# geoHeil/splink

Hardware: AMD Instinct MI355X
Metric: candidate pairs scored/sec (gammas+E+M per iter) (higher is better)
Workload: dtype fp64; 1 GPU; cfg2: synthetic person-record dedupe, 1M x sqrt(N) records, blocking surname|dob, 5 comparison columns (JW-3 x2, exact-2 x2, Levenshtein-3); records=1000000, candidate_pairs=45981122, comparison_columns=5, candidate_ordinals_total=46222173, comparison_windows=2, parallelism=pair-ordinal shards x1, RCCL all-reduce of pattern histogram

## Files before the change

### include/splink_hip.h

```cpp
#ifndef SPLINK_HIP_H
#define SPLINK_HIP_H

#include <stdint.h>

#ifdef __cplusplus
extern "C" {
#endif

#define SPK_OK 0
#define SPK_E_INVALID (-1)
#define SPK_E_HIP (-2)
#define SPK_E_OOM (-3)
#define SPK_E_STATE (-4)
#define SPK_E_LIMIT (-5)

#define SPK_LINK_DEDUPE 0
#define SPK_LINK_ONLY 1
#define SPK_LINK_AND_DEDUPE 2

typedef struct spk_ctx spk_ctx;

const char *spk_last_error(void);
int spk_version(void);
int spk_device_count(int *out);
// ... 100 lines not shown
                       const int32_t *rule_program, int shard, int n_shards, int n_cols,
                       const spk_column_program *cols, int n_when, const int32_t *when_first_instr,
                       const int32_t *when_n_instr, const int32_t *when_level, int n_instr,
                       const spk_instr *instr, int n_operands, const spk_operand *operands, int n_lits,
                       const int64_t *lit_offsets, const uint8_t *lit_utf8, int64_t *out_n_pairs,
                       int64_t *out_n_candidates_total);
int spk_block_residual_info(spk_ctx *ctx, int64_t *out_enumerated, double *out_filter_ms);
int spk_gammas_copy(spk_ctx *ctx, int64_t start, int64_t count, int8_t *out);
int spk_gammas_load(spk_ctx *ctx, int n_cols, const int32_t *n_levels, int64_t n, const int8_t *gammas);
int spk_n_patterns(spk_ctx *ctx, int64_t *out);
int spk_gammas_deferred(spk_ctx *ctx, int64_t *out);
int spk_gammas_exact_counts(spk_ctx *ctx, int64_t *out, int n);
int spk_gammas_exact_ms(spk_ctx *ctx, double *out, int n);
int spk_gammas_exact_list(spk_ctx *ctx, int k, int32_t *out, int64_t n);
int spk_gammas_implied_pairs(spk_ctx *ctx, int64_t *out, int n);
int spk_gammas_set_simple(spk_ctx *ctx, int on);
int spk_gammas_simple_count(spk_ctx *ctx, int *out);
int spk_gammas_set_window(spk_ctx *ctx, int64_t pairs);
int spk_gammas_windows(spk_ctx *ctx, int64_t *out);
int spk_gammas_set_streams(spk_ctx *ctx, int streams, int64_t min_pairs);
int spk_gammas_set_graph(spk_ctx *ctx, int on);
int spk_gammas_graph_launches(spk_ctx *ctx, int64_t *out);
int spk_gammas_set_lev_kernel(spk_ctx *ctx, int mode);
int spk_gammas_view_regions(spk_ctx *ctx, int64_t *out);

int spk_jaro_winkler_sim(spk_ctx *ctx, int64_t n, const int64_t *l_offsets, const uint8_t *l_utf8,
                         const int64_t *r_offsets, const uint8_t *r_utf8, double *out);
int spk_levenshtein(spk_ctx *ctx, int64_t n, const int64_t *l_offsets, const uint8_t *l_utf8,
                    const int64_t *r_offsets, const uint8_t *r_utf8, double *out);

int spk_em_iteration(spk_ctx *ctx, double lambda, double one_minus, const double *m, const double *u,
                     double *out_stats, int n_stats);
int spk_em_iteration_start(spk_ctx *ctx, double lambda, double one_minus, const double *m, const double *u,
                           int n_stats);
int spk_em_iteration_wait(spk_ctx *ctx, double *out_stats, int n_stats);
int spk_em_histogram(spk_ctx *ctx, uint64_t *d_hist);
int spk_em_set_lane_histogram(spk_ctx *ctx, int on);
int spk_em_finalize(spk_ctx *ctx, const uint64_t *d_hist, double lambda, double one_minus, const double *m,
                    const double *u, double *out_stats, int n_stats);
int spk_em_histogram_async(spk_ctx *ctx, uint64_t *d_hist);
int spk_em_finalize_start(spk_ctx *ctx, const uint64_t *d_hist, double lambda, double one_minus, const double *m,
                          const double *u, int n_stats);
int spk_score(spk_ctx *ctx, double lambda, double one_minus, const double *m, const double *u, int64_t start,
              int64_t count, double *out_mp);

#define SPK_SEL_MP 0
// ... 58 lines not shown
```

### splink_amd/_native.py

```python
from __future__ import annotations

import ctypes
import os

import numpy as np

_HERE = os.path.dirname(os.path.abspath(__file__))
LIB_PATH = os.environ.get("SPLINK_AMD_LIB", os.path.join(_HERE, "libsplink_hip.so"))

SPK_OK = 0
SPK_E_INVALID = -1
SPK_E_HIP = -2
SPK_E_OOM = -3
SPK_E_STATE = -4
SPK_E_LIMIT = -5

LINK_TYPES = {"dedupe_only": 0, "link_only": 1, "link_and_dedupe": 2}

OPERAND_DTYPE = np.dtype([("kind", "<i4"), ("side", "<i4"), ("col", "<i4"), ("lit", "<i4"), ("num", "<f8"),
                          ("has_num_default", "<i4"), ("substr_start", "<i4"), ("substr_len", "<i4"),
                          ("pad", "<i4")], align=True)
INSTR_DTYPE = np.dtype([("op", "<i4"), ("a", "<i4"), ("b", "<i4"), ("cmp", "<i4"), ("i0", "<i4"), ("pad", "<i4"),
                        ("t", "<f8")], align=True)
PROGRAM_DTYPE = np.dtype([("n_levels", "<i4"), ("else_level", "<i4"), ("n_when", "<i4"), ("first_when", "<i4")],
# ... 10 lines not shown
SELECT_CHUNK = 2048
COMPONENTS_CHUNK = 1024
assert OPERAND_DTYPE.itemsize == 40 and INSTR_DTYPE.itemsize == 32 and PROGRAM_DTYPE.itemsize == 16

OP = {"ISNULL": 1, "NOTNULL": 2, "STR_CMP": 3, "NUM_CMP": 4, "JW": 5, "LEV": 6, "LEVRATIO": 7, "ABSDIFF": 8,
      "PERCDIFF": 9, "CONST": 10, "LEN": 11, "AND": 20, "OR": 21, "NOT": 22}
CMP = {"=": 0, "==": 0, "!=": 1, "<>": 1, "<": 2, "<=": 3, ">": 4, ">=": 5}

EXPORTS = [
    "spk_last_error", "spk_version", "spk_device_count", "spk_ctx_create", "spk_ctx_destroy", "spk_ctx_set_stream",
    "spk_ctx_sync", "spk_ctx_set_link_type", "spk_ctx_kernel_ms", "spk_ctx_enable_timing", "spk_table_create",
    "spk_table_add_utf8", "spk_table_add_float64", "spk_table_set_rank", "spk_table_set_key", "spk_block",
    "spk_pairs_count", "spk_pairs_copy", "spk_pairs_load", "spk_gammas", "spk_gammas_copy", "spk_gammas_load",
    "spk_n_patterns", "spk_gammas_deferred", "spk_em_histogram", "spk_em_finalize", "spk_em_iteration", "spk_score",
    "spk_tf_accumulate", "spk_tf_apply", "spk_jaro_winkler_sim", "spk_levenshtein", "spk_gammas_exact_counts",
    "spk_gammas_set_simple", "spk_gammas_exact_list", "spk_gammas_simple_count", "spk_em_set_lane_histogram", "spk_table_set_rank_null",
    "spk_gammas_view_regions", "spk_ctx_lds_per_block", "spk_ctx_memory", "spk_raw_utf8", "spk_raw_i64", "spk_key_build", "spk_rank_from_raw", "spk_cluster", "spk_table_add_raw_utf8",
    "spk_gammas_implied_pairs", "spk_tf_column_values", "spk_tf_accumulate_column", "spk_tf_apply_columns", "spk_tf_copy", "spk_tf_set_mode",
    "spk_tf_accumulate_exact", "spk_tf_accumulate_column_exact", "spk_tf_limbs_to_sum", "spk_tf_scales",
    "spk_tf_scales_column", "spk_raw_utf8_arrow", "spk_raw_utf8_arrow_chunks", "spk_table_digest", "spk_raw_release",
    "spk_em_iteration_start", "spk_em_iteration_wait", "spk_ctx_kernel_ms_done", "spk_em_histogram_async",
    "spk_em_finalize_start", "spk_gammas_exact_ms", "spk_gammas_set_window", "spk_gammas_windows", "spk_gammas_set_streams", "spk_gammas_set_graph",
    "spk_gammas_graph_launches",
    "spk_gammas_set_lev_kernel",
    "spk_block_residual", "spk_block_residual_info",
    "spk_select", "spk_select_copy", "spk_select_info", "spk_select_release",
    "spk_components", "spk_components_edges", "spk_components_copy", "spk_components_info", "spk_components_release",
]
TF_LIMBS = 14


class NativeUnavailable(RuntimeError):
    """libsplink_hip.so or a gfx950 HIP device is unavailable (there is no CPU fallback)."""


_lib = None


def load_library():
    global _lib
    if _lib is not None:
        return _lib
    if not os.path.exists(LIB_PATH):
        raise NativeUnavailable(f"{LIB_PATH} not found: build it with `python -c 'import __graft_entry__ as g; g.build()'`")
    lib = ctypes.CDLL(LIB_PATH)
    lib.spk_last_error.restype = ctypes.c_char_p
    lib.spk_ctx_destroy.restype = None
# ... 309 lines not shown
    def gammas_set_window(self, pairs: int):
        check(self._lib.spk_gammas_set_window(self._h, ctypes.c_int64(int(pairs))), "spk_gammas_set_window")

    def gammas_set_streams(self, streams: int, min_pairs: int = 1 << 22):
        check(self._lib.spk_gammas_set_streams(self._h, ctypes.c_int(int(streams)), ctypes.c_int64(int(min_pairs))),
              "spk_gammas_set_streams")

    def gammas_set_graph(self, on: bool):
        check(self._lib.spk_gammas_set_graph(self._h, ctypes.c_int(1 if on else 0)), "spk_gammas_set_graph")

    def gammas_graph_launches(self) -> int:
        n = ctypes.c_int64(0)
        check(self._lib.spk_gammas_graph_launches(self._h, ctypes.byref(n)), "spk_gammas_graph_launches")
        return n.value

    def gammas_windows(self) -> int:
        n = ctypes.c_int64(0)
        check(self._lib.spk_gammas_windows(self._h, ctypes.byref(n)), "spk_gammas_windows")
        return n.value

    def gammas_set_lev_kernel(self, mode: int):
        check(self._lib.spk_gammas_set_lev_kernel(self._h, ctypes.c_int(int(mode))), "spk_gammas_set_lev_kernel")

    def lds_per_block(self) -> int:
        n = ctypes.c_int(0)
        check(self._lib.spk_ctx_lds_per_block(self._h, ctypes.byref(n)), "spk_ctx_lds_per_block")
        return n.value

    MEMORY_PARTS = ("raw_columns", "record_encodings", "row_images", "pairs", "codes", "work_lists", "em_score_tf",
                    "total")

    def memory(self) -> dict:
        out = np.zeros(8, dtype=np.int64)
        check(self._lib.spk_ctx_memory(self._h, _ptr(out)), "spk_ctx_memory")
        return dict(zip(self.MEMORY_PARTS, [int(x) for x in out]))

    def gammas_view_regions(self) -> int:
        n = ctypes.c_int64(0)
        check(self._lib.spk_gammas_view_regions(self._h, ctypes.byref(n)), "spk_gammas_view_regions")
        return n.value

    def gammas_exact_ms(self, n: int):
        out = np.zeros(max(n, 1), dtype=np.float64)
        check(self._lib.spk_gammas_exact_ms(self._h, _ptr(out), ctypes.c_int(n)), "spk_gammas_exact_ms")
        return out[:n].tolist()

# ... 237 lines not shown
```

### splink_amd/csrc/spk_ctx.hip

```cpp
#include <algorithm>
#include <cstring>

#include "spk_internal.h"

namespace spk {

static thread_local std::string g_last_error;
void set_error(const std::string &msg) { g_last_error = msg; }

Table::~Table() {
    for (Column *c : cols) delete c;
    for (int w = 0; w < 2; ++w)
        for (DevBuf<int64_t> *k : key[w]) delete k;
}

int ensure_desc(spk_ctx *ctx, Table &t) {
    if (!t.desc_dirty && t.d_desc.p) return SPK_OK;
    std::vector<ColDesc> h(t.cols.size());
    for (size_t i = 0; i < t.cols.size(); ++i) {
        Column *c = t.cols[i];
        ColDesc d{};
        d.kind = c ? c->kind : COL_NONE;
        if (c && c->kind == COL_STR) {
            d.units = c->units.p;
            d.meta = c->meta.p;
            d.planes = c->planes.p;
            d.planes_hi = c->planes_hi.n ? c->planes_hi.p : nullptr;
            d.bag = c->bag.n ? c->bag.p : nullptr;
        } else if (c && c->kind == COL_NUM) {
            d.val = c->val.p;
            d.valid = c->valid.p;
        }
        h[i] = d;
    }
    SPK_TRY(t.d_desc.alloc(h.size() ? h.size() : 1));
    if (!h.empty())
        SPK_HIP(hipMemcpyAsync(t.d_desc.p, h.data(), h.size() * sizeof(ColDesc), hipMemcpyHostToDevice, ctx->stream));
    SPK_HIP(hipStreamSynchronize(ctx->stream));
    t.desc_dirty = false;
    return SPK_OK;
}


__global__ void k_utf8_decode(int64_t n, const int64_t *__restrict__ off8, const int64_t *__restrict__ src_off,
                              const int32_t *__restrict__ perm, const uint8_t *__restrict__ bytes,
                              const uint8_t *__restrict__ valid, uint16_t *__restrict__ units,
                              RecMeta *__restrict__ meta, uint64_t *__restrict__ planes,
                              uint64_t *__restrict__ planes_hi, const int64_t *__restrict__ ids) {
    int64_t row = (int64_t)blockIdx.x * blockDim.x + threadIdx.x;
    if (row >= n) return;
    const int64_t src = perm ? (int64_t)perm[row] : row;
// ... 174 lines not shown
            }
            const int sh = (b & 7) * 4;
            const uint32_t x = w[b >> 3];
            if (((x >> sh) & 15u) < 15u) w[b >> 3] = x + (1u << sh);
        }
        w[7] |= (other << 16) | ((uint32_t)len << 24);
    } else {
        w[7] = 0xFF000000u;
    }
    bag[2 * row] = make_uint4(w[0], w[1], w[2], w[3]);
    bag[2 * row + 1] = make_uint4(w[4], w[5], w[6], w[7]);
}

int build_bag_rows(spk_ctx *ctx, int64_t n, Column *c) {
    SPK_TRY(c->bag.alloc((size_t)(2 * n + 2)));
    if (n > 0) {
        k_bag_rows<<<(unsigned)((n + BAG_THREADS - 1) / BAG_THREADS), BAG_THREADS, 0, ctx->stream>>>(n, c->meta.p,
                                                                                                  c->units.p, c->bag.p);
        SPK_HIP(hipGetLastError());
    }
    return SPK_OK;
}

int launch_unit_bits(spk_ctx *ctx, int64_t n, Column *c) {
    c->unit_bits = false;
    c->bag.release();
    if (n <= 0) return SPK_OK;
    DevBuf<unsigned int> d;
    SPK_TRY(d.alloc(2));
    const unsigned int init[2] = {0u, 0xFFu};
    SPK_HIP(hipMemcpyAsync(d.p, init, sizeof(init), hipMemcpyHostToDevice, ctx->stream));
    const int64_t blocks = std::min<int64_t>((n + 255) / 256, 4 * (int64_t)ctx->n_cu);
    k_unit_bits<<<(unsigned)blocks, 256, 0, ctx->stream>>>(n, c->meta.p, c->planes.p, c->planes_hi.p, d.p);
    SPK_HIP(hipGetLastError());
    unsigned int h[2];
    SPK_HIP(hipMemcpyAsync(h, d.p, sizeof(h), hipMemcpyDeviceToHost, ctx->stream));
    SPK_HIP(hipStreamSynchronize(ctx->stream));
    c->unit_or = h[0];
    c->unit_and = h[1];
    c->unit_bits = true;
    return SPK_OK;
}

int launch_utf8_decode(spk_ctx *ctx, int64_t n, const int64_t *off8, const int64_t *src_off, const int32_t *perm,
                       const uint8_t *bytes, const uint8_t *valid, Column *c, bool long_rows, const int64_t *ids) {
    if (n <= 0) return SPK_OK;
    k_utf8_decode<<<(unsigned)((n + 255) / 256), 256, 0, ctx->stream>>>(n, off8, src_off, perm, bytes, valid, c->units.p,
                                                                        c->meta.p, c->planes.p,
                                                                        long_rows ? c->planes_hi.p : nullptr, ids);
// ... 428 lines not shown
```

### splink_amd/csrc/spk_filter.hip

```cpp
#include <algorithm>
#include <cmath>
#include <cstring>

#include "spk_gamma.h"

namespace spk {

enum LevKind : int32_t { LK_GE = 0, LK_LE = 1, LK_EXACT = 2, LK_RATIO = 3 };

struct FCommon {
    int64_t p0, p1;
    uint32_t in;
    uint32_t stride;
    int32_t k;
    int32_t null_level;
    int64_t imp_lo, imp_hi;
    uint32_t imp_add;
    int32_t und_same;
    int ws;
};

struct FEq {
    FCommon c;
    int32_t lv_same, lv_diff;
    int32_t eq4;
};

struct FJw {
    FCommon c;
    int64_t h0, h1;
    int32_t lv_one, lv_zero, lv_bound;
    float cf;
    int32_t geq;
    FEq ge[2];
};

struct FLev {
    FCommon c;
    int32_t lv_same, lv_same_empty, lv_else;
    int32_t n;
    int32_t kind[MAX_TESTS], a[MAX_TESTS], cmp[MAX_TESTS], level[MAX_TESTS];
    double t[MAX_TESTS];
};

struct FNum {
    FCommon c;
    int32_t null_level, else_level, n_tests;
    int32_t op[MAX_TESTS], cmp[MAX_TESTS], level[MAX_TESTS];
    double t[MAX_TESTS];
};

struct FiltArgs {
    const int32_t *pl, *pr;
    const uint8_t *img0, *img1;
    uint32_t plane0, plane1;
    void *codes;
    int32_t *work;
    unsigned int *region_count;
    int64_t P, region_len;
    int n_regions, region_base;
    const int16_t *thr;
    int n_thr;
    int nj, nl, ne, nn;
// ... 136 lines not shown
#pragma unroll
    for (int u = 0; u < FP; ++u) {
        const bool sat = lf[u] >= LEN_SAT || ls[u] >= LEN_SAT;
        const bool exact = same[u] || zero[u];
        const uint32_t add = same[u] ? (lf[u] > 0 ? a_one : a_zero) : (zero[u] ? a_zero : a_bound);
        const bool u0 = (same[u] && und_same) || sat || (!exact && hi[u] >= J.cf);
        und[u] = act[u] && !nul[u] && u0;
        acc[u] += und[u] ? 0u : (nul[u] ? a_null : add);
    }
}
template <int FP>
__device__ __attribute__((always_inline)) inline void f_jw(const FiltArgs &A, const FJw &J, const uint32_t (&ox)[FP],
                                                           const uint32_t (&oy)[FP], const bool (&act)[FP],
                                                           uint32_t (&acc)[FP], bool (&und)[FP]) {
    JwData<FP> d;
    ld_jw<FP>(A, J, ox, oy, d);
    ev_jw<FP>(J, d, act, acc, und);
}

template <int FP>
struct Data16 {
    uint4 a[FP], b[FP];
};
template <int FP>
__device__ __attribute__((always_inline)) inline void ev_lev(const FLev &L, const int16_t *s_thr, const Data16<FP> &d,
                                                             const bool (&act)[FP], uint32_t (&acc)[FP], bool (&und)[FP]) {
    const uint4(&a)[FP] = d.a;
    const uint4(&b)[FP] = d.b;
    bool same[FP], nul[FP], bmp[FP], u0[FP];
    int lo[FP], hi[FP], S[FP];
    bool need = false;
#pragma unroll
    for (int u = 0; u < FP; ++u) {
        same[u] = a[u].x == b[u].x && a[u].y == b[u].y;
        nul[u] = a[u].y == LENS_NULL || b[u].y == LENS_NULL;
        const int la = lens_u16(a[u].y), lb = lens_u16(b[u].y), na = lens_cp(a[u].y), nb = lens_cp(b[u].y);
        u0[u] = (same[u] && L.c.und_same) || la >= LEN_SAT || lb >= LEN_SAT || na >= LEN_SAT || nb >= LEN_SAT;
        bmp[u] = na == la && nb == lb && !same[u] && !nul[u];
        need = need || bmp[u];
        lo[u] = na > nb ? na - nb : nb - na;
        hi[u] = na > nb ? na : nb;
        S[u] = na + nb;
    }
    if (__any(need)) {
#pragma unroll
        for (int u = 0; u < FP; ++u) {
            const int na = lens_cp(a[u].y), nb = lens_cp(b[u].y);
            const int bag = hi[u] - sketch_inter_ub_bf(img_sketch(a[u]), img_sketch(b[u]), na, nb);
            lo[u] = (bmp[u] && bag > lo[u]) ? bag : lo[u];
        }
    }
    Chain ch[FP];
#pragma unroll
    for (int u = 0; u < FP; ++u) ch[u] = Chain(L.lv_else);
    bool fast = (L.n == 1 || L.n == 2) && L.kind[0] == LK_RATIO && L.a[0] >= 0 &&
                (L.n == 1 || (L.kind[1] == LK_RATIO && L.a[1] >= 0));
    if (fast) {
        bool narrow = true;
#pragma unroll
        for (int u = 0; u < FP; ++u) narrow = narrow && S[u] < THR_S;
        fast = !__any(!narrow);
    }
    if (fast) {
        const int a0 = L.a[0], lv0 = L.level[0];
#pragma unroll
// ... 305 lines not shown
    common(s, A, s.off, J.c);
    J.h0 = (int64_t)(s.off2 >> 4) * A.img_rows0 * 16;
    J.h1 = (int64_t)(s.off2 >> 4) * A.img_rows1 * 16;
    auto first_pass = [&](double v) {
        for (int i = 0; i < s.n_tests; ++i)
            if (hcmp(v, s.t[i], s.cmp[i])) return s.level[i];
        return s.else_level;
    };
    J.lv_one = first_pass(1.0);
    J.lv_zero = first_pass(0.0);
    J.lv_bound = s.else_level;
    J.cf = INFINITY;
    for (int i = 0; i < s.n_tests; ++i) {
        if (hcmp(0.0, s.t[i], s.cmp[i])) {
            J.lv_bound = s.level[i];
            break;
        }
        J.cf = std::min(J.cf, s.jw_cf[i]);
    }
}

static void make_lev(const SimpleCol &s, const GammaArgs &A, FLev &L) {
    common(s, A, s.off, L.c);
    auto same_level = [&](bool empty) {
        for (int i = 0; i < s.n_tests; ++i) {
            const int op = s.op[i];
            bool r;
            if (op == SPK_OP_STR_CMP) r = s.cmp[i] == SPK_CMP_EQ;
            else if (op == SPK_OP_LEV) r = hcmp(0.0, s.t[i], s.cmp[i]);
            else r = !empty && hcmp(0.0, s.t[i], s.cmp[i]);
            if (r) return s.level[i];
        }
        return s.else_level;
    };
    L.lv_same = same_level(false);
    L.lv_same_empty = same_level(true);
    L.n = 0;
    L.lv_else = s.else_level;
    for (int i = 0; i < s.n_tests; ++i) {
        const int op = s.op[i];
        if (op == SPK_OP_STR_CMP) {
            if (s.cmp[i] == SPK_CMP_EQ) continue;
            L.lv_else = s.level[i];
            break;
        }
        const int n = L.n++;
// ... 102 lines not shown
```

### splink_amd/csrc/spk_gamma.h

```cpp
#pragma once

#include <vector>

#include "spk_strsim.h"

namespace spk {

constexpr int F_THREADS = 256;
constexpr int X_THREADS = 256;
constexpr int U_THREADS = 128;

enum Mode { M_FILTER = 0, M_EXACT = 1, M_SLOW = 2, M_HUGE = 3 };
enum Status { ST_DONE = 0, ST_UNDECIDED = 1, ST_NEEDS_SLOW = 2 };

constexpr int MAX_TESTS = 6;
constexpr int MAX_SIMPLE = 64;
enum SimpleKind : int32_t { SK_STR = 1, SK_NUM = 2 };
enum SimpleClass : int32_t { SC_NONE = 0, SC_EQ = 1, SC_JW = 2, SC_LEV = 3, SC_NUM = 4 };
struct SimpleCol {
    int32_t k;
    int32_t kind;
    int32_t col;
    int32_t null_level, else_level, n_tests;
    int32_t op[MAX_TESTS], cmp[MAX_TESTS], level[MAX_TESTS];
    double t[MAX_TESTS];
    int64_t stride;
    int32_t cls;
    int32_t off;
    int32_t off2;
    int32_t has_ids;
    int32_t eq4;
    int32_t tflag[MAX_TESTS];
    int32_t lev_a[MAX_TESTS];
    float jw_cf[MAX_TESTS];
    int64_t imp_lo, imp_hi;
    int32_t eq_level;
    int32_t thr_off[MAX_TESTS];
    int32_t np;
};
constexpr int THR_S = 256;
constexpr int32_t TF_ZERO = 1;
constexpr int32_t TF_ONE = 2;
constexpr int32_t TF_GE = 4;
constexpr int32_t TF_EXACT = 8;
constexpr int32_t TF_EQ = 16;

constexpr int IMG_MAX = 256;
constexpr int64_t VIEW_MIN_IMAGE_BYTES = (int64_t)192 << 20;
constexpr uint32_t LENS_NULL = 0xFFFFFFFFu;
constexpr int LEN_SAT = 0xFFFE;
typedef uint32_t u32x4_t __attribute__((ext_vector_type(4)));
typedef uint32_t u32x2_t __attribute__((ext_vector_type(2)));
__device__ inline __amdgpu_buffer_rsrc_t image_rsrc(const uint8_t *base, int64_t bytes) {
    return __builtin_amdgcn_make_buffer_rsrc((void *)base, (short)0, (int)bytes, 0x00020000);
}
constexpr int64_t IMG_MAX_ROWS = ((int64_t)1 << 27) - 1;

__host__ __device__ inline int64_t img_at(int64_t rows, int64_t row, int off) {
    return ((int64_t)(off >> 4) * rows + row) * 16 + (off & 15);
}

// ... 205 lines not shown
```

### splink_amd/csrc/spk_gamma.hip

```cpp
#include <chrono>
#include <cstdio>
#include <algorithm>
#include <cstring>
#include <type_traits>
#include <cmath>

#include "spk_gamma.h"

namespace spk {

__device__ inline void apply_substr(StrView &s, int pos, int len) {
    int nc = s.ncp;
    int start = pos > 0 ? pos - 1 : (pos < 0 ? nc + pos : 0);
    long end = (long)start + len;
    if (start < 0) start = 0;
    if (end > nc) end = nc;
    s.has_meta = 0;
    s.planes = nullptr;
    if (start >= end) {
        s.n = 0;
        s.ncp = 0;
        return;
    }
    if (s.ncp == s.n) {
// ... 314 lines not shown
            }
        }
        if (r == KU) return ST_UNDECIDED;
        if (r == KT) {
            level = sc.level[i];
            return ST_DONE;
        }
    }
    level = sc.else_level;
    return ST_DONE;
}

__global__ void k_build_image(int64_t n, const ColDesc *__restrict__ cols, const SimpleCol *__restrict__ simple,
                              int n_simple, uint8_t *__restrict__ img, int64_t rows_img) {
    const int64_t row = (int64_t)blockIdx.x * blockDim.x + threadIdx.x;
    if (row >= n) return;
    for (int j = 0; j < n_simple; ++j) {
        const SimpleCol &sc = simple[j];
        const ColDesc &c = cols[sc.col];
        if (sc.cls == SC_NUM) {
            const bool ok = c.valid[row] != 0;
            *reinterpret_cast<double *>(img + img_at(rows_img, row, sc.off)) = ok ? c.val[row] : 0.0;
            *reinterpret_cast<uint2 *>(img + img_at(rows_img, row, sc.off + 8)) = make_uint2(ok ? 1u : 0u, 0u);
            continue;
        }
        const RecMeta m = c.meta[row];
        uint32_t lens = LENS_NULL;
        if (m.len16 >= 0) {
            const int l16 = m.len16 < LEN_SAT ? m.len16 : LEN_SAT;
            const int lcp = meta_cplen(m) < LEN_SAT ? meta_cplen(m) : LEN_SAT;
            lens = (uint32_t)l16 | ((uint32_t)lcp << 16);
        }
        if (sc.eq4) {
            *reinterpret_cast<uint32_t *>(img + img_at(rows_img, row, sc.off)) = m.len16 < 0 ? 0xFFFFFFFFu : m.key;
            continue;
        }
        *reinterpret_cast<uint2 *>(img + img_at(rows_img, row, sc.off)) = make_uint2(m.key, lens);
        if (sc.cls != SC_EQ) *reinterpret_cast<uint64_t *>(img + img_at(rows_img, row, sc.off + 8)) = m.sketch;
        if (sc.cls == SC_JW) *reinterpret_cast<uint64_t *>(img + img_at(rows_img, row, sc.off2)) = m.head;
    }
}

__global__ __launch_bounds__(F_THREADS) void k_gamma_filter(GammaArgs A) {
    __shared__ unsigned int s_cnt[MAX_SIMPLE];
    for (int i = threadIdx.x; i < A.n_complex; i += F_THREADS) s_cnt[i] = 0;
    __syncthreads();
// ... 1538 lines not shown
    return SPK_OK;
}

static int build_images(spk_ctx *ctx, Table &t0, Table &t1, GammaArgs &A, int64_t stride,
                        const std::vector<SimpleCol> &simple) {
    A.img0 = A.img1 = nullptr;
    A.img_stride = stride;
    if (stride <= 0 || A.n_simple == 0) return SPK_OK;
    Table *ts[2] = {&t0, &t1};
    for (int s = 0; s < 2; ++s) {
        if (s == 1 && &t1 == &t0) {
            A.img1 = A.img0;
            A.img_rows1 = A.img_rows0;
            break;
        }
        Table &t = *ts[s];
        std::vector<int64_t> key = {(int64_t)t.version, t.n, stride};
        for (const SimpleCol &sc : simple) {
            key.push_back(sc.cls);
            key.push_back(sc.col);
            key.push_back(sc.off);
            key.push_back(sc.off2);
            key.push_back(sc.eq4);
        }
        const bool fresh = ctx->img[s].p && ctx->img_key[s] == key;
        SPK_TRY(ctx->img[s].alloc((size_t)(t.n + 1) * (size_t)stride));
        ctx->img_key[s] = key;
        if (t.n > 0 && !fresh) {
            k_build_image<<<(unsigned)((t.n + 255) / 256), 256, 0, ctx->stream>>>(t.n, t.d_desc.p, A.simple, A.n_simple,
                                                                                 ctx->img[s].p, t.n + 1);
            SPK_HIP(hipGetLastError());
        }
        (s == 0 ? A.img0 : A.img1) = ctx->img[s].p;
        (s == 0 ? A.img_rows0 : A.img_rows1) = t.n + 1;
    }
    return SPK_OK;
}

static bool classify_simple(int k, const spk_column_program &prog, const int32_t *wf, const int32_t *wn,
                            const int32_t *wl, const spk_instr *instr, const spk_operand *ops, const Table &t0,
                            const Table &t1, const std::vector<int64_t> &stride, SimpleCol *out) {
    if (prog.n_when < 1 || prog.n_when - 1 > MAX_TESTS) return false;
    const int w0 = prog.first_when;
    if (wn[w0] != 3) return false;
    const spk_instr *n = instr + wf[w0];
    if (n[0].op != SPK_OP_ISNULL || n[1].op != SPK_OP_ISNULL || n[2].op != SPK_OP_OR) return false;
// ... 449 lines not shown
            const uint32_t all = t0.cols[sc.col]->unit_and & t1.cols[sc.col]->unit_and;
            while (sc.np > 5 && (((any ^ all) >> (sc.np - 1)) & 1u) == 0) --sc.np;
        }
        sc.has_ids = (t0.cols[sc.col]->has_ids && t1.cols[sc.col]->has_ids) ? 1 : 0;
        implied_equal(ctx, t0, t1, sc);
    }
    if (ctx->lev_bag) {
        bool built[2] = {false, false};
        for (const SimpleCol &sc : simple) {
            if (sc.cls != SC_LEV || sc.kind != SK_STR || !t0.cols[sc.col]->planes_hi.n || !t1.cols[sc.col]->planes_hi.n)
                continue;
            for (int s = 0; s < 2; ++s) {
                Table &t = s ? t1 : t0;
                Column *c = t.cols[sc.col];
                if (c->kind != COL_STR || c->bag.n || t.n <= 0) continue;
                SPK_TRY(build_bag_rows(ctx, t.n, c));
                t.desc_dirty = true;
                built[s] = true;
            }
        }
        if (built[0]) SPK_TRY(ensure_desc(ctx, t0));
        if (built[1]) SPK_TRY(ensure_desc(ctx, t1));
    }
    std::vector<int16_t> thr_tab;
    for (SimpleCol &sc : simple) {
        for (int i = 0; i < MAX_TESTS; ++i) sc.thr_off[i] = -1;
        if (sc.cls != SC_LEV) continue;
        for (int i = 0; i < sc.n_tests; ++i) {
            if (sc.op[i] != SPK_OP_LEVRATIO || (sc.cmp[i] != SPK_CMP_LE && sc.cmp[i] != SPK_CMP_LT)) continue;
            sc.thr_off[i] = (int32_t)thr_tab.size();
            for (int S = 0; S < THR_S; ++S) {
                int th = -1;
                const double den = (double)S / 2.0;
                for (int v = 0; v < THR_S && S > 0; ++v)
                    if (host_cmp((double)v / den, sc.t[i], sc.cmp[i])) th = v;
                    else break;
                thr_tab.push_back((int16_t)th);
            }
        }
    }
    const int64_t img_stride = layout_image(simple);
    for (size_t i = 0; i < simple.size();) {
        if (simple[i].cls == SC_NONE) {
            complex_k.push_back(simple[i].k);
            simple.erase(simple.begin() + (long)i);
        } else {
// ... 143 lines not shown
        for (const Column *c : t->cols)
            if (c && c->kind == COL_STR) G.max_units = std::max<int64_t>(G.max_units, c->max_bytes);
    for (int i = 0; i < n_lits; ++i) G.max_units = std::max<int64_t>(G.max_units, llen[i]);

    ctx->exact_carry.clear();
    ctx->deferred_carry = 0;
    ctx->last_windows = n_win;
    ctx->last_split = split;
    ctx->split_w = split ? W : 0;
    SPK_TRY(ctx->begin(K_GAMMA));
    ViewLaunch V{};
    bool have_view = false;
    ctx->last_view_regions = 0;
    if (P > 0) {
        SPK_TRY(build_images(ctx, t0, t1, A, img_stride, simple));
        const bool big = (A.img_rows0 + A.img_rows1) * img_stride > VIEW_MIN_IMAGE_BYTES;
        if ((ctx->use_views == 1 && big) || ctx->use_views == 2) SPK_TRY(build_view_images(ctx, A, img_stride, &V, &have_view));
    }
    std::vector<int64_t> gkey;
    {
        auto ptr = [](const void *q) { return (int64_t)(uintptr_t)q; };
        gkey = {P, n_win, split ? 1 : 0, W, K, ctx->code_bytes, (int64_t)ctx->pairs_epoch, (int64_t)ctx->table_epoch,
                (int64_t)std::hash<std::string>()(std::string(blob.begin(), blob.end())), ctx->lev_kernel,
                ctx->lev_bag ? 1 : 0, ctx->filter_mode, ctx->use_views, ctx->slow_force_skip ? 1 : 0,
                have_view ? 1 : 0, ptr(ctx->stream), ptr(ctx->codes.p), ptr(ctx->pl.p), ptr(ctx->pr.p), ptr(ctx->pvl.p),
                ptr(ctx->prog_blob.p), ptr(ctx->img[0].p), ptr(ctx->img[1].p), ptr(ctx->work.p), ptr(ctx->xlist.p),
                ptr(ctx->xinfo.p), ptr(ctx->xpref.p), ptr(ctx->region_count.p), ctx->xcap, ptr(ctx->alt.work.p),
                ptr(ctx->alt.xlist.p), ptr(ctx->alt.xinfo.p), ptr(ctx->alt.xpref.p), ptr(ctx->alt.region_count.p),
                ctx->alt.xcap, ptr(ctx->alt.stream), ctx->slow_seen_valid ? 1 : 0, (int64_t)ctx->timing};
        for (uint8_t f : ctx->slow_seen) gkey.push_back(f);
        for (int v = 0; v < MAX_VIEWS; ++v) gkey.push_back(ptr(ctx->vimg[v][0].p));
    }
    const bool graphable = ctx->use_graph && !ctx->timing_exact && P > 0 && fresh_blob && (split || n_win == 1);
    const bool replay = graphable && ctx->gexec && gkey == ctx->gkey;
    const bool capture = graphable && !replay && gkey == ctx->gkey_prev;
    ctx->gkey_prev = gkey;
    if (split && !replay) {
        if (!ctx->alt.gplan) ctx->alt.gplan = new GammaPlan();
        *ctx->alt.gplan = G;
    }
    bool via_graph = replay;
    if (replay) {
        ctx->gplan->slow_skipped = ctx->gskip0;
        if (split) ctx->alt.gplan->slow_skipped = ctx->gskip1;
        ctx->last_view_regions = ctx->gview_regions;
        SPK_HIP(hipGraphLaunch(ctx->gexec, ctx->stream));
        ++ctx->graph_launches;
// ... 411 lines not shown
}

extern "C" int spk_gammas_set_simple(spk_ctx *ctx, int on) {
    SPK_REQUIRE(ctx && on >= 0 && on % 10 <= 1 && on % 100 < 30 && on < 200, SPK_E_INVALID,
                "spk_gammas_set_simple: mode 0, 1 (+10 / +20) (+100)");
    ctx->use_views = on % 100 >= 20 ? 2 : (on % 100 >= 10 ? 0 : 1);
    ctx->filter_mode = on % 10;
    ctx->slow_force_skip = on >= 100;
    return SPK_OK;
}

extern "C" int spk_ctx_memory(spk_ctx *ctx, int64_t *out8) {
    SPK_REQUIRE(ctx && out8, SPK_E_INVALID, "spk_ctx_memory: null arg");
    auto b = [](const auto &buf) { return (int64_t)(buf.n * sizeof(*buf.p)); };
    int64_t m[8] = {0, 0, 0, 0, 0, 0, 0, 0};
    for (const RawCol *r : ctx->raw)
        if (r) m[0] += b(r->off) + b(r->bytes) + b(r->i64) + b(r->valid);
    for (const Table &t : ctx->table) {
        m[1] += b(t.perm) + b(t.rank) + b(t.d_desc);
        for (int w = 0; w < 2; ++w)
            for (const DevBuf<int64_t> *k : t.key[w])
                if (k) m[1] += b(*k);
        for (const Column *c : t.cols)
            if (c) m[1] += b(c->units) + b(c->meta) + b(c->planes) + b(c->planes_hi) + b(c->bag) + b(c->val) + b(c->valid);
    }
    for (int s = 0; s < 2; ++s) {
        m[2] += b(ctx->img[s]);
        for (int v = 0; v < MAX_VIEWS; ++v) m[2] += b(ctx->vimg[v][s]);
    }
    m[3] = b(ctx->pl) + b(ctx->pr) + b(ctx->pvl) + b(ctx->pvr);
    for (int v = 0; v < MAX_VIEWS; ++v) m[3] += b(ctx->views[v].rowsL) + b(ctx->views[v].rowsR);
    m[4] = b(ctx->codes);
    m[5] = b(ctx->work) + b(ctx->xlist) + b(ctx->xpref) + b(ctx->xinfo) + b(ctx->region_count) + b(ctx->prog_blob) +
           b(ctx->alt.work) + b(ctx->alt.xlist) + b(ctx->alt.xpref) + b(ctx->alt.xinfo) + b(ctx->alt.region_count);
    m[6] = b(ctx->hist) + b(ctx->mpat) + b(ctx->llpat) + b(ctx->cpat) + b(ctx->stats) + b(ctx->mu) + b(ctx->em_ticket) +
           b(ctx->em_row) + b(ctx->em_hot) + b(ctx->mp) + b(ctx->mpat_score) + b(ctx->tf_uniq) + b(ctx->tf_runs) +
           b(ctx->tf_nruns) + b(ctx->tf_mp) + b(ctx->tf_hist) +
           b(ctx->tf_sort) +
           b(ctx->sel.ord) + b(ctx->sel.l) + b(ctx->sel.r) + b(ctx->sel.code) + b(ctx->sel.mpat) +
           b(ctx->comp.label);
    for (int i = 0; i < 7; ++i) m[7] += m[i];
    for (int i = 0; i < 8; ++i) out8[i] = m[i];
    return SPK_OK;
}

extern "C" int spk_ctx_lds_per_block(spk_ctx *ctx, int *out) {
    SPK_REQUIRE(ctx && out, SPK_E_INVALID, "null arg");
// ... 34 lines not shown

extern "C" int spk_gammas_set_streams(spk_ctx *ctx, int streams, int64_t min_pairs) {
    SPK_REQUIRE(ctx && (streams == 1 || streams == 2) && min_pairs >= 0, SPK_E_INVALID,
                "spk_gammas_set_streams: 1 or 2 streams, min_pairs >= 0");
    SPK_TRY(settle_gammas(ctx, nullptr));
    ctx->gamma_streams = streams;
    ctx->split_min = min_pairs;
    return SPK_OK;
}

extern "C" int spk_gammas_windows(spk_ctx *ctx, int64_t *out) {
    SPK_REQUIRE(ctx && out, SPK_E_INVALID, "spk_gammas_windows: bad args");
    *out = ctx->last_windows;
    return SPK_OK;
}

extern "C" int spk_gammas_set_lev_kernel(spk_ctx *ctx, int mode) {
    SPK_REQUIRE(ctx && mode >= 0 && mode <= 3, SPK_E_INVALID, "spk_gammas_set_lev_kernel: mode 0 .. 3");
    ctx->lev_kernel = mode == 3 ? 2 : mode;
    ctx->lev_bag = mode != 3;
    return SPK_OK;
}

#ifdef SPK_LEVQ_STATS
extern "C" int spk_debug_levq_stats(uint64_t *out, int reset) {
    SPK_HIP(hipDeviceSynchronize());
    SPK_HIP(hipMemcpyFromSymbol(out, HIP_SYMBOL(g_levq), sizeof(uint64_t) * 16));
    if (reset) {
        static const unsigned long long zero[16] = {};
        SPK_HIP(hipMemcpyToSymbol(HIP_SYMBOL(g_levq), zero, sizeof(zero)));
    }
    return SPK_OK;
}
#endif
```

### splink_amd/csrc/spk_internal.h

```cpp
#pragma once

#include <hip/hip_runtime.h>

#include <cstdint>
#include <string>
#include <utility>
#include <vector>

#include "../../include/splink_hip.h"

namespace spk {

void set_error(const std::string &msg);

#define SPK_HIP(expr)                                                                         \
    do {                                                                                      \
        hipError_t _e = (expr);                                                               \
        if (_e != hipSuccess) {                                                               \
            ::spk::set_error(std::string(#expr) + ": " + hipGetErrorString(_e));              \
            return _e == hipErrorOutOfMemory ? SPK_E_OOM : SPK_E_HIP;                         \
        }                                                                                     \
    } while (0)

#define SPK_REQUIRE(cond, code, msg)                                                          \
// ... 28 lines not shown
__host__ __device__ inline int32_t meta_cplen(const RecMeta &m) { return (int32_t)(m.cpf & 0xFFFFFFu); }
__host__ __device__ inline int64_t meta_off(const RecMeta &m) { return (int64_t)m.off4 * 4; }

constexpr int N_PLANES = 8;

__host__ __device__ inline uint32_t sketch_bucket(uint32_t u) {
    if (u < 128u) {
        if (u >= 'a' && u <= 'z') return u - 'a';
        if (u >= 'A' && u <= 'Z') return u - 'A';
        if (u >= '0' && u <= '9') return 26u + (u - '0') % 3u;
        return 29u + u % 3u;
    }
    return ((u * 2654435761u) >> 16) & 31u;
}

__host__ __device__ inline void sketch_add(uint64_t &sk, uint32_t unit) {
    const uint32_t b = sketch_bucket(unit);
    const uint64_t lo = 1ull << b, hi = 1ull << (32 + b);
    if ((sk & lo) && (sk & hi)) return;
    if (sk & lo) sk = (sk & ~lo) | hi;
    else sk |= lo;
}

struct ColDesc {
    int32_t kind;
    int32_t pad;
    const uint16_t *units;
    const RecMeta *meta;
    const uint64_t *planes;
    const uint64_t *planes_hi;
    const uint4 *bag;
    const double *val;
    const uint8_t *valid;
};

template <typename T>
struct DevBuf {
    T *p = nullptr;
    size_t n = 0;
    int alloc(size_t count) {
        if (count <= n && p) return SPK_OK;
        release();
        if (count == 0) return SPK_OK;
        hipError_t e = hipMalloc(&p, count * sizeof(T));
        if (e != hipSuccess) {
            p = nullptr;
            set_error(std::string("hipMalloc failed: ") + hipGetErrorString(e));
            return e == hipErrorOutOfMemory ? SPK_E_OOM : SPK_E_HIP;
        }
        n = count;
        return SPK_OK;
    }
    void release() {
        if (p) (void)hipFree(p);
// ... 6 lines not shown
    DevBuf &operator=(const DevBuf &) = delete;
    DevBuf(DevBuf &&o) noexcept : p(o.p), n(o.n) {
        o.p = nullptr;
        o.n = 0;
    }
    DevBuf &operator=(DevBuf &&o) noexcept {
        if (this != &o) {
            release();
            std::swap(p, o.p);
            std::swap(n, o.n);
        }
        return *this;
    }
};

struct Column {
    ColKind kind = COL_NONE;
    DevBuf<uint16_t> units;
    int64_t units_len = 0;
    DevBuf<RecMeta> meta;
    DevBuf<uint64_t> planes;
    DevBuf<uint64_t> planes_hi;
    DevBuf<uint4> bag;
    DevBuf<double> val;
    DevBuf<uint8_t> valid;
    bool has_ids = false;
    int64_t max_bytes = 0;
    uint64_t src[2] = {0, 0};
    bool has_empty = false;
    int64_t n_ids = -1;
    bool unit_bits = false;
    uint32_t unit_or = 0, unit_and = 0xFFu;
};

struct KeyTerm {
    uint64_t src_l = 0, src_r = 0;
    bool plain = false;
};

enum RawKind : int32_t { RAW_UTF8 = 1, RAW_I64 = 2 };
struct RawCol {
    RawKind kind = RAW_UTF8;
    uint64_t serial = 0;
    bool has_empty = false;
    int64_t n = 0;
    int64_t max_len = 0;
// ... 119 lines not shown
        h_info_n = 0;
        if (hipHostMalloc(reinterpret_cast<void **>(&h_info), n * 8, hipHostMallocDefault) != hipSuccess) {
            h_info = nullptr;
            spk::set_error("hipHostMalloc failed");
            return SPK_E_OOM;
        }
        h_info_n = n;
        return SPK_OK;
    }
    spk::DevBuf<uint8_t> img[2];
    std::vector<int64_t> img_key[2];
    spk::DevBuf<uint8_t> vimg[spk::MAX_VIEWS][2];
    std::vector<int64_t> vimg_key[spk::MAX_VIEWS][2];
    uint64_t table_epoch = 0;
    spk::DevBuf<uint8_t> prog_blob;
    std::vector<uint8_t> last_blob;
    spk::GammaPlan *gplan = nullptr;
    void (*gplan_free)(spk::GammaPlan *) = nullptr;
    bool gamma_pending = false;
    std::vector<uint8_t> slow_seen;
    bool slow_seen_valid = false;
    bool lev_bag = true;
    int lev_kernel = 2;
    bool slow_force_skip = false;
    uint64_t slow_key_pairs = 0, slow_key_tables = 0;
    spk::DevBuf<unsigned int> region_count;

    struct Slot {
        spk::DevBuf<int32_t> work, xlist;
        spk::DevBuf<int64_t> xpref, xinfo;
        spk::DevBuf<unsigned int> region_count;
        int64_t xcap = 0;
        int64_t *h_info = nullptr;
        size_t h_info_n = 0;
        hipEvent_t ev_info = nullptr;
        spk::GammaPlan *gplan = nullptr;
        bool gamma_pending = false;
        hipStream_t stream = nullptr;
        std::vector<hipEvent_t> xev0, xev1;
        std::vector<char> xev_used;
    } alt;
    int gamma_streams = 2;
    int64_t split_min = (int64_t)1 << 22;
    hipEvent_t ev_fork = nullptr, ev_join = nullptr;
    bool split_ready = false;
    bool use_graph = false;
// ... 72 lines not shown
    bool timing_exact = false;
    hipEvent_t ev0[2][spk::K_COUNT] = {}, ev1[2][spk::K_COUNT] = {};
    bool ev_used[2][spk::K_COUNT] = {};
    int ev_slot[spk::K_COUNT] = {};

    std::vector<hipEvent_t> xev0, xev1;
    std::vector<char> xev_used;
    int xbegin(int k);
    int xend(int k);

    int begin(spk::Kern k);
    int end(spk::Kern k);
    spk::Table &side_table(int operand_side) { return table[(operand_side == 1 && link_type == SPK_LINK_ONLY) ? 1 : 0]; }
};

namespace spk {
int ensure_desc(spk_ctx *ctx, Table &t);
int settle_gammas(spk_ctx *ctx, bool *fixed);
int em_requeue(spk_ctx *ctx);
int pattern_mp_table(spk_ctx *ctx, double lambda, double one_minus, const double *m, const double *u, double *d_mpat);
int new_column(spk_ctx *ctx, int side, int col, Column **out);
int launch_unit_bits(spk_ctx *ctx, int64_t n, Column *c);
int build_bag_rows(spk_ctx *ctx, int64_t n, Column *c);
int launch_utf8_decode(spk_ctx *ctx, int64_t n, const int64_t *off8, const int64_t *src_off, const int32_t *perm,
                       const uint8_t *bytes, const uint8_t *valid, Column *c, bool long_rows, const int64_t *ids);
}
```

Baseline: 49.66 billion pairs/s.

## Add per-row positional multiset signatures for Levenshtein lower-bound filtering

Builds a per-record 128-bit signature holding the string length and two-bit-saturating bucket counts (30 character buckets) for each half of the string. The Levenshtein filter then computes a stronger lower bound from length gap, whole-string bag distance and a split-half bound, so more pairs can be resolved without running the exact DP. The mode is on by default for non-free-text string Levenshtein columns. It adds a preprocessing kernel, extra per-row memory and more ALU work per pair, and it drops the 'same' and bitmap fast paths when this mode is active.

```diff
diff --git a/include/splink_hip.h b/include/splink_hip.h
--- a/include/splink_hip.h
+++ b/include/splink_hip.h
@@ -146,6 +146,7 @@
 int spk_gammas_set_graph(spk_ctx *ctx, int on);
 int spk_gammas_graph_launches(spk_ctx *ctx, int64_t *out);
 int spk_gammas_set_lev_kernel(spk_ctx *ctx, int mode);
+int spk_gammas_set_lev_bound(spk_ctx *ctx, int mode);
 int spk_gammas_view_regions(spk_ctx *ctx, int64_t *out);
 
 int spk_jaro_winkler_sim(spk_ctx *ctx, int64_t n, const int64_t *l_offsets, const uint8_t *l_utf8,
diff --git a/splink_amd/_native.py b/splink_amd/_native.py
--- a/splink_amd/_native.py
+++ b/splink_amd/_native.py
@@ -56,7 +56,7 @@
     "spk_em_iteration_start", "spk_em_iteration_wait", "spk_ctx_kernel_ms_done", "spk_em_histogram_async",
     "spk_em_finalize_start", "spk_gammas_exact_ms", "spk_gammas_set_window", "spk_gammas_windows", "spk_gammas_set_streams", "spk_gammas_set_graph",
     "spk_gammas_graph_launches",
-    "spk_gammas_set_lev_kernel",
+    "spk_gammas_set_lev_kernel", "spk_gammas_set_lev_bound",
     "spk_block_residual", "spk_block_residual_info",
     "spk_select", "spk_select_copy", "spk_select_info", "spk_select_release",
     "spk_components", "spk_components_edges", "spk_components_copy", "spk_components_info", "spk_components_release",
@@ -412,6 +412,9 @@
     def gammas_set_lev_kernel(self, mode: int):
         check(self._lib.spk_gammas_set_lev_kernel(self._h, ctypes.c_int(int(mode))), "spk_gammas_set_lev_kernel")
 
+    def gammas_set_lev_bound(self, mode: int):
+        check(self._lib.spk_gammas_set_lev_bound(self._h, ctypes.c_int(int(mode))), "spk_gammas_set_lev_bound")
+
     def lds_per_block(self) -> int:
         n = ctypes.c_int(0)
         check(self._lib.spk_ctx_lds_per_block(self._h, ctypes.byref(n)), "spk_ctx_lds_per_block")
diff --git a/splink_amd/csrc/spk_ctx.hip b/splink_amd/csrc/spk_ctx.hip
--- a/splink_amd/csrc/spk_ctx.hip
+++ b/splink_amd/csrc/spk_ctx.hip
@@ -27,6 +27,7 @@
             d.planes = c->planes.p;
             d.planes_hi = c->planes_hi.n ? c->planes_hi.p : nullptr;
             d.bag = c->bag.n ? c->bag.p : nullptr;
+            d.pos = c->pos.n ? c->pos.p : nullptr;
         } else if (c && c->kind == COL_NUM) {
             d.val = c->val.p;
             d.valid = c->valid.p;
@@ -247,9 +248,48 @@
     return SPK_OK;
 }
 
+__global__ void k_pos_rows(int64_t n, const RecMeta *__restrict__ meta, const uint16_t *__restrict__ units,
+                           uint4 *__restrict__ pos) {
+    const int64_t row = (int64_t)blockIdx.x * blockDim.x + threadIdx.x;
+    if (row >= n) return;
+    const RecMeta m = meta[row];
+    const int len = m.len16;
+    if (len < 0 || len >= (int)POS_NONE || meta_cplen(m) != len) {
+        pos[row] = make_uint4(len < 0 ? POS_NULL : POS_NONE, 0u, 0u, 0u);
+        return;
+    }
+    const uint16_t *u = units + meta_off(m);
+    const int half = (len + 1) >> 1;
+    uint32_t lo[2] = {0u, 0u}, hi[2] = {0u, 0u};
+#pragma unroll
+    for (int h = 0; h < 2; ++h) {
+        uint32_t l = 0u, g = 0u;
+        for (int i = h ? half : 0; i < (h ? len : half); ++i) {
+            const uint32_t bit = 1u << pos_bucket(u[i]);
+            if (l & g & bit) continue;
+            g |= l & bit;
+            l ^= bit;
+        }
+        lo[h] = l;
+        hi[h] = g;
+    }
+    pos[row] = make_uint4((uint32_t)len | (lo[0] << 8), (lo[0] >> 24) | (hi[0] << 6), (hi[0] >> 26) | (lo[1] << 4),
+                          (lo[1] >> 28) | (hi[1] << 2));
+}
+
+int build_pos_rows(spk_ctx *ctx, int64_t n, Column *c) {
+    SPK_TRY(c->pos.alloc((size_t)(n + 1)));
+    if (n > 0) {
+        k_pos_rows<<<(unsigned)((n + 255) / 256), 256, 0, ctx->stream>>>(n, c->meta.p, c->units.p, c->pos.p);
+        SPK_HIP(hipGetLastError());
+    }
+    return SPK_OK;
+}
+
 int launch_unit_bits(spk_ctx *ctx, int64_t n, Column *c) {
     c->unit_bits = false;
     c->bag.release();
+    c->pos.release();
     if (n <= 0) return SPK_OK;
     DevBuf<unsigned int> d;
     SPK_TRY(d.alloc(2));
diff --git a/splink_amd/csrc/spk_filter.hip b/splink_amd/csrc/spk_filter.hip
--- a/splink_amd/csrc/spk_filter.hip
+++ b/splink_amd/csrc/spk_filter.hip
@@ -39,6 +39,7 @@
     FCommon c;
     int32_t lv_same, lv_same_empty, lv_else;
     int32_t n;
+    int32_t pos;
     int32_t kind[MAX_TESTS], a[MAX_TESTS], cmp[MAX_TESTS], level[MAX_TESTS];
     double t[MAX_TESTS];
 };
@@ -221,6 +222,41 @@
 struct Data16 {
     uint4 a[FP], b[FP];
 };
+
+struct PosRow {
+    int n;
+    uint32_t l1, h1, l2, h2;
+};
+__device__ __attribute__((always_inline)) inline PosRow pos_unpack(const uint4 &v) {
+    PosRow r;
+    r.n = (int)(v.x & 0xFFu);
+    r.l1 = __builtin_amdgcn_alignbit(v.y, v.x, 8) & POS_MASK;
+    r.h1 = __builtin_amdgcn_alignbit(v.z, v.y, 6) & POS_MASK;
+    r.l2 = __builtin_amdgcn_alignbit(v.w, v.z, 4) & POS_MASK;
+    r.h2 = v.w >> 2;
+    return r;
+}
+__device__ __attribute__((always_inline)) inline int pos_sum(uint32_t l, uint32_t h) {
+    return __builtin_popcount(l) + 2 * __builtin_popcount(h);
+}
+__device__ __attribute__((always_inline)) inline int pos_inter(uint32_t aL, uint32_t aH, uint32_t bL, uint32_t bH,
+                                                               int la, int lb) {
+    const uint32_t gt = (aH & ~bH) | (~(aH ^ bH) & aL & ~bL);
+    const uint32_t mL = (aL & ~gt) | (bL & gt), mH = (aH & ~gt) | (bH & gt);
+    const int ea = la - pos_sum(aL, aH), eb = lb - pos_sum(bL, bH);
+    return pos_sum(mL, mH) + (ea < eb ? ea : eb);
+}
+__device__ __attribute__((always_inline)) inline void pos_whole(const PosRow &r, uint32_t &wL, uint32_t &wH) {
+    const uint32_t hh = r.h1 | r.h2, ll = r.l1 | r.l2;
+    wH = hh | (r.l1 & r.l2);
+    wL = ((r.l1 ^ r.l2) & ~hh) | (r.h1 & r.h2) | (hh & ll);
+}
+__device__ __attribute__((always_inline)) inline int pos_side(int Ax, int Bx, int Ix, int Ay, int By, int Iy) {
+    const int d1 = Ax - Bx, d2 = By - Ay, d3 = Ax - Ix, d4 = By - Iy;
+    int d = min(max(d1, d2), min(d3, d4));
+    d = min(max(d, 0), By);
+    return max(max(d3 - d, Bx - Ix), d - d1) + max(max(d4 - d, Ay - Iy), d - d2);
+}
 template <int FP>
 __device__ __attribute__((always_inline)) inline void ev_lev(const FLev &L, const int16_t *s_thr, const Data16<FP> &d,
                                                              const bool (&act)[FP], uint32_t (&acc)[FP], bool (&und)[FP]) {
@@ -229,17 +265,41 @@
     bool same[FP], nul[FP], bmp[FP], u0[FP];
     int lo[FP], hi[FP], S[FP];
     bool need = false;
-#pragma unroll
-    for (int u = 0; u < FP; ++u) {
-        same[u] = a[u].x == b[u].x && a[u].y == b[u].y;
-        nul[u] = a[u].y == LENS_NULL || b[u].y == LENS_NULL;
-        const int la = lens_u16(a[u].y), lb = lens_u16(b[u].y), na = lens_cp(a[u].y), nb = lens_cp(b[u].y);
-        u0[u] = (same[u] && L.c.und_same) || la >= LEN_SAT || lb >= LEN_SAT || na >= LEN_SAT || nb >= LEN_SAT;
-        bmp[u] = na == la && nb == lb && !same[u] && !nul[u];
-        need = need || bmp[u];
-        lo[u] = na > nb ? na - nb : nb - na;
-        hi[u] = na > nb ? na : nb;
-        S[u] = na + nb;
+    if (L.pos) {
+#pragma unroll
+        for (int u = 0; u < FP; ++u) {
+            const PosRow x = pos_unpack(a[u]), y = pos_unpack(b[u]);
+            const int na = x.n, nb = y.n;
+            nul[u] = na == (int)POS_NULL || nb == (int)POS_NULL;
+            const bool none = na >= (int)POS_NONE || nb >= (int)POS_NONE;
+            same[u] = false;
+            bmp[u] = false;
+            hi[u] = na > nb ? na : nb;
+            S[u] = none ? 0 : na + nb;
+            const int A1 = (na + 1) >> 1, A2 = na >> 1, B1 = (nb + 1) >> 1, B2 = nb >> 1;
+            const int I1 = pos_inter(x.l1, x.h1, y.l1, y.h1, A1, B1), I2 = pos_inter(x.l2, x.h2, y.l2, y.h2, A2, B2);
+            uint32_t awL, awH, bwL, bwH;
+            pos_whole(x, awL, awH);
+            pos_whole(y, bwL, bwH);
+            const int bag = hi[u] - pos_inter(awL, awH, bwL, bwH, na, nb);
+            const int seg = min(pos_side(A1, B1, I1, A2, B2, I2), pos_side(A2, B2, I2, A1, B1, I1));
+            const int gap = na > nb ? na - nb : nb - na;
+            lo[u] = max(max(gap, bag), seg);
+            u0[u] = none || lo[u] == 0;
+        }
+    } else {
+#pragma unroll
+        for (int u = 0; u < FP; ++u) {
+            same[u] = a[u].x == b[u].x && a[u].y == b[u].y;
+            nul[u] = a[u].y == LENS_NULL || b[u].y == LENS_NULL;
+            const int la = lens_u16(a[u].y), lb = lens_u16(b[u].y), na = lens_cp(a[u].y), nb = lens_cp(b[u].y);
+            u0[u] = (same[u] && L.c.und_same) || la >= LEN_SAT || lb >= LEN_SAT || na >= LEN_SAT || nb >= LEN_SAT;
+            bmp[u] = na == la && nb == lb && !same[u] && !nul[u];
+            need = need || bmp[u];
+            lo[u] = na > nb ? na - nb : nb - na;
+            hi[u] = na > nb ? na : nb;
+            S[u] = na + nb;
+        }
     }
     if (__any(need)) {
 #pragma unroll
@@ -591,6 +651,7 @@
 
 static void make_lev(const SimpleCol &s, const GammaArgs &A, FLev &L) {
     common(s, A, s.off, L.c);
+    L.pos = s.pos;
     auto same_level = [&](bool empty) {
         for (int i = 0; i < s.n_tests; ++i) {
             const int op = s.op[i];
diff --git a/splink_amd/csrc/spk_gamma.h b/splink_amd/csrc/spk_gamma.h
--- a/splink_amd/csrc/spk_gamma.h
+++ b/splink_amd/csrc/spk_gamma.h
@@ -37,6 +37,7 @@
     int32_t eq_level;
     int32_t thr_off[MAX_TESTS];
     int32_t np;
+    int32_t pos;
 };
 constexpr int THR_S = 256;
 constexpr int32_t TF_ZERO = 1;
diff --git a/splink_amd/csrc/spk_gamma.hip b/splink_amd/csrc/spk_gamma.hip
--- a/splink_amd/csrc/spk_gamma.hip
+++ b/splink_amd/csrc/spk_gamma.hip
@@ -360,6 +360,10 @@
             const bool ok = c.valid[row] != 0;
             *reinterpret_cast<double *>(img + img_at(rows_img, row, sc.off)) = ok ? c.val[row] : 0.0;
             *reinterpret_cast<uint2 *>(img + img_at(rows_img, row, sc.off + 8)) = make_uint2(ok ? 1u : 0u, 0u);
+            continue;
+        }
+        if (sc.cls == SC_LEV && sc.pos) {
+            *reinterpret_cast<uint4 *>(img + img_at(rows_img, row, sc.off)) = c.pos[row];
             continue;
         }
         const RecMeta m = c.meta[row];
@@ -1944,6 +1948,7 @@
             key.push_back(sc.off);
             key.push_back(sc.off2);
             key.push_back(sc.eq4);
+            key.push_back(sc.pos);
         }
         const bool fresh = ctx->img[s].p && ctx->img_key[s] == key;
         SPK_TRY(ctx->img[s].alloc((size_t)(t.n + 1) * (size_t)stride));
@@ -2439,6 +2444,24 @@
         if (built[0]) SPK_TRY(ensure_desc(ctx, t0));
         if (built[1]) SPK_TRY(ensure_desc(ctx, t1));
     }
+    {
+        bool built[2] = {false, false};
+        for (SimpleCol &sc : simple) {
+            const bool free_text = sc.kind == SK_STR && t0.cols[sc.col]->planes_hi.n && t1.cols[sc.col]->planes_hi.n;
+            sc.pos = (sc.cls == SC_LEV && sc.kind == SK_STR && ctx->lev_bound == 1 && !free_text) ? 1 : 0;
+            if (!sc.pos) continue;
+            for (int s = 0; s < 2; ++s) {
+                Table &t = s ? t1 : t0;
+                Column *c = t.cols[sc.col];
+                if (c->kind != COL_STR || c->pos.n || t.n <= 0) continue;
+                SPK_TRY(build_pos_rows(ctx, t.n, c));
+                t.desc_dirty = true;
+                built[s] = true;
+            }
+        }
+        if (built[0]) SPK_TRY(ensure_desc(ctx, t0));
+        if (built[1]) SPK_TRY(ensure_desc(ctx, t1));
+    }
     std::vector<int16_t> thr_tab;
     for (SimpleCol &sc : simple) {
         for (int i = 0; i < MAX_TESTS; ++i) sc.thr_off[i] = -1;
@@ -2628,7 +2651,7 @@
         auto ptr = [](const void *q) { return (int64_t)(uintptr_t)q; };
         gkey = {P, n_win, split ? 1 : 0, W, K, ctx->code_bytes, (int64_t)ctx->pairs_epoch, (int64_t)ctx->table_epoch,
                 (int64_t)std::hash<std::string>()(std::string(blob.begin(), blob.end())), ctx->lev_kernel,
-                ctx->lev_bag ? 1 : 0, ctx->filter_mode, ctx->use_views, ctx->slow_force_skip ? 1 : 0,
+                ctx->lev_bag ? 1 : 0, ctx->lev_bound, ctx->filter_mode, ctx->use_views, ctx->slow_force_skip ? 1 : 0,
                 have_view ? 1 : 0, ptr(ctx->stream), ptr(ctx->codes.p), ptr(ctx->pl.p), ptr(ctx->pr.p), ptr(ctx->pvl.p),
                 ptr(ctx->prog_blob.p), ptr(ctx->img[0].p), ptr(ctx->img[1].p), ptr(ctx->work.p), ptr(ctx->xlist.p),
                 ptr(ctx->xinfo.p), ptr(ctx->xpref.p), ptr(ctx->region_count.p), ctx->xcap, ptr(ctx->alt.work.p),
@@ -3086,7 +3109,9 @@
             for (const DevBuf<int64_t> *k : t.key[w])
                 if (k) m[1] += b(*k);
         for (const Column *c : t.cols)
-            if (c) m[1] += b(c->units) + b(c->meta) + b(c->planes) + b(c->planes_hi) + b(c->bag) + b(c->val) + b(c->valid);
+            if (c)
+                m[1] += b(c->units) + b(c->meta) + b(c->planes) + b(c->planes_hi) + b(c->bag) + b(c->pos) + b(c->val) +
+                        b(c->valid);
     }
     for (int s = 0; s < 2; ++s) {
         m[2] += b(ctx->img[s]);
@@ -3167,6 +3192,12 @@
     return SPK_OK;
 }
 
+extern "C" int spk_gammas_set_lev_bound(spk_ctx *ctx, int mode) {
+    SPK_REQUIRE(ctx && (mode == 0 || mode == 1), SPK_E_INVALID, "spk_gammas_set_lev_bound: mode 0 or 1");
+    ctx->lev_bound = mode;
+    return SPK_OK;
+}
+
 #ifdef SPK_LEVQ_STATS
 extern "C" int spk_debug_levq_stats(uint64_t *out, int reset) {
     SPK_HIP(hipDeviceSynchronize());
diff --git a/splink_amd/csrc/spk_internal.h b/splink_amd/csrc/spk_internal.h
--- a/splink_amd/csrc/spk_internal.h
+++ b/splink_amd/csrc/spk_internal.h
@@ -74,6 +74,16 @@
     else sk |= lo;
 }
 
+constexpr int POS_BUCKETS = 30;
+constexpr uint32_t POS_MASK = (1u << POS_BUCKETS) - 1u;
+constexpr uint32_t POS_NULL = 255u, POS_NONE = 254u;
+__host__ __device__ inline uint32_t pos_bucket(uint32_t u) {
+    if (u >= 'a' && u <= 'z') return u - 'a';
+    if (u >= 'A' && u <= 'Z') return u - 'A';
+    if (u >= '0' && u <= '9') return 26u + (u & 1u);
+    return 28u + ((u >> 1) & 1u);
+}
+
 struct ColDesc {
     int32_t kind;
     int32_t pad;
@@ -82,6 +92,7 @@
     const uint64_t *planes;
     const uint64_t *planes_hi;
     const uint4 *bag;
+    const uint4 *pos;
     const double *val;
     const uint8_t *valid;
 };
@@ -134,6 +145,7 @@
     DevBuf<uint64_t> planes;
     DevBuf<uint64_t> planes_hi;
     DevBuf<uint4> bag;
+    DevBuf<uint4> pos;
     DevBuf<double> val;
     DevBuf<uint8_t> valid;
     bool has_ids = false;
@@ -299,6 +311,7 @@
     bool slow_seen_valid = false;
     bool lev_bag = true;
     int lev_kernel = 2;
+    int lev_bound = 1;
     bool slow_force_skip = false;
     uint64_t slow_key_pairs = 0, slow_key_tables = 0;
     spk::DevBuf<unsigned int> region_count;
@@ -417,6 +430,7 @@
 int new_column(spk_ctx *ctx, int side, int col, Column **out);
 int launch_unit_bits(spk_ctx *ctx, int64_t n, Column *c);
 int build_bag_rows(spk_ctx *ctx, int64_t n, Column *c);
+int build_pos_rows(spk_ctx *ctx, int64_t n, Column *c);
 int launch_utf8_decode(spk_ctx *ctx, int64_t n, const int64_t *off8, const int64_t *src_off, const int32_t *perm,
                        const uint8_t *bytes, const uint8_t *valid, Column *c, bool long_rows, const int64_t *ids);
 }
```

Measured after the change: 53.74 billion pairs/s (median of 6 runs). +8.2%, better.
